# latticeboltzmann/2d-lb

Hardware: AMD Instinct MI355X
Metric: MLUPS (million lattice updates per second), fused D2Q9 BGK step (higher is better)
Workload: dtype f32

## Files before the change

### 2d-lb_amd/csrc/kernels_deep2.h

```cpp
#pragma once

namespace {

constexpr int deep2_split(int D) { return D >= 8 ? 4 : (D + 1) / 2; }
constexpr int deep2_rw_front(int D) { return deep2_split(D) - 2 >= 2 ? 2 : 1; }
constexpr int deep2_rw_back(int D) { return (D - deep2_split(D) + 1) - 2 >= 2 ? 2 : 1; }
constexpr int DEEP2_WAVES = 4;

__device__ __forceinline__ void deep2_barrier() { asm volatile("s_waitcnt lgkmcnt(0)\n\ts_barrier" ::: "memory"); }

__device__ __forceinline__ void deep2_set_prio(const StepArgs &a, const int role_mode)
{
    int mode = a.deep2_prio;
#ifdef LB_DIAG
    if ((a.diag >> 25) & 3) mode = ((a.diag >> 25) & 3) - 1;
#endif
    if (mode == role_mode) __builtin_amdgcn_s_setprio(1);
}

template <int BC, bool MASK, int F, int RW, bool DOWN, int NST>
__device__ __forceinline__ void deep2_front_fill(const StepArgs &a, const DeepCtx &cx, DeepState<RW, F - 1 - RW> &st, Row1 &ra, Row1 &rb,
                                                 int &trip)
{
    if constexpr (NST < F) {
        deep2_barrier();
        if (trip < cx.n_iter) {
            if ((NST & 1) == 0) deep_iter<BC, MASK, false, F, RW, 1, DOWN, NST, -1, DEEP_FRONT>(a, cx, NST - 1, st, rb, ra);
            else deep_iter<BC, MASK, false, F, RW, 1, DOWN, NST, -1, DEEP_FRONT>(a, cx, NST - 1, st, ra, rb);
        }
        deep2_barrier();
        ++trip;
        deep2_front_fill<BC, MASK, F, RW, DOWN, NST + 1>(a, cx, st, ra, rb, trip);
    }
}

template <int BC, bool MASK, int D, int F, int RW, bool DOWN>
__device__ __forceinline__ void deep2_front(const StepArgs &a, const int x0, const int ym, const int len, const int trips, f4a (*mine)[64],
                                            f4a (*other)[64], f4a (*ho)[64], f4a (*dma)[64])
{
    deep2_set_prio(a, 1);
    DeepCtx cx;
    cx.lane = threadIdx.x;
    const int xr = x0 + cx.lane * 4;
    cx.x4 = skirt_column<BC>(a, xr, deep_skirt_lanes(D));
    cx.store_lane = false;
    cx.ym = ym; cx.n_iter = len + D - 1;
    cx.mine = mine; cx.other = other; cx.ho = ho; cx.dma = dma;
    cx.dma_off = __builtin_amdgcn_readfirstlane((unsigned)reinterpret_cast<unsigned long long>(dma));
    DeepState<RW, F - 1 - RW> st = {};
    auto row_at = [&](int p) { return DOWN ? ym - 1 - p : ym + p; };
    Row1 ra, rb;
    deep_row_issue_lds<BC, MASK>(a, row_at(0), cx.x4, cx.dma_off, ra);
    int trip = 0;
    deep2_front_fill<BC, MASK, F, RW, DOWN, 1>(a, cx, st, ra, rb, trip);
    if ((F - 1) & 1) ra = rb;
    for (; trip < trips; ++trip) {
#ifdef LB_DIAG
        if (!(a.diag & (1 << 24)))
#endif
        deep2_barrier();
        if (trip < cx.n_iter) {
            deep_iter<BC, MASK, false, F, RW, 1, DOWN, F, -1, DEEP_FRONT>(a, cx, trip, st, ra, rb);
            ra = rb;
        }
#ifdef LB_DIAG
        if (!(a.diag & (1 << 24)))
#endif
        deep2_barrier();
    }
    asm volatile("s_waitcnt vmcnt(0)" ::: "memory");
}

template <bool MASK>
__device__ __forceinline__ void deep2_take(const DeepCtx &cx, Row1 &cur)
{
#pragma unroll
    for (int k = 0; k < 9; ++k) cur.q[k] = cx.ho[k][cx.lane];
    cur.mk = uc4{0, 0, 0, 0};
    if (MASK) cur.mk = __builtin_bit_cast(uc4, reinterpret_cast<const unsigned *>(cx.ho[9])[cx.lane]);
    cur.have = true;
}

template <int BC, bool MASK, bool MACRO, int DB, int RW, bool DOWN, int NST>
__device__ __forceinline__ void deep2_back_fill(const StepArgs &a, const DeepCtx &cx, DeepState<RW, DB - 1 - RW> &st, Row1 &cur, int &j)
{
    if constexpr (NST < DB) {
        if (j < cx.n_iter) deep2_take<MASK>(cx, cur);
        deep2_barrier();
        if (j < cx.n_iter) deep_iter<BC, MASK, MACRO, DB, RW, 0, DOWN, NST, -1, DEEP_BACK>(a, cx, NST - 1, st, cur, cur);
        deep2_barrier();
        ++j;
        deep2_back_fill<BC, MASK, MACRO, DB, RW, DOWN, NST + 1>(a, cx, st, cur, j);
    }
}

template <int BC, bool MASK, bool MACRO, int D, int F, int RW, bool DOWN>
__device__ __forceinline__ void deep2_back(const StepArgs &a, const int x0, const int ym, const int len, const int trips, f4a (*mine)[64],
                                           f4a (*other)[64], f4a (*ho)[64])
{
    constexpr int DB = D - F + 1;
    deep2_set_prio(a, 2);
    DeepCtx cx;
    cx.lane = threadIdx.x;
    const int xr = x0 + cx.lane * 4;
    cx.x4 = skirt_column<BC>(a, xr, deep_skirt_lanes(D));
    cx.store_lane = skirt_store_lane(a, cx.lane, xr, deep_skirt_lanes(D));
    cx.ym = ym; cx.n_iter = len + DB - 1;
    cx.mine = mine; cx.other = other; cx.ho = ho;
    DeepState<RW, DB - 1 - RW> st = {};
    Row1 cur;
    cur.wp = WrapPatch{0.f, 0.f, 0.f, 0.f, 0.f, 0.f};
    cur.hsolid = false; cur.hxc = -1; cur.rr = 0;
    for (int t = 0; t < F; ++t) {
        deep2_barrier();
        deep2_barrier();
    }
    int j = 0;
    deep2_back_fill<BC, MASK, MACRO, DB, RW, DOWN, 1>(a, cx, st, cur, j);
    for (; j + F < trips; ++j) {
        if (j < cx.n_iter) deep2_take<MASK>(cx, cur);
#ifdef LB_DIAG
        if (!(a.diag & (1 << 24)))
#endif
        deep2_barrier();
        if (j < cx.n_iter) deep_iter<BC, MASK, MACRO, DB, RW, 0, DOWN, DB, -1, DEEP_BACK>(a, cx, j, st, cur, cur);
#ifdef LB_DIAG
        if (!(a.diag & (1 << 24)))
#endif
        deep2_barrier();
    }
}

template <int BC, bool MASK, bool MACRO, int D>
__global__ __launch_bounds__(64 * DEEP2_WAVES, 2) void k_deep2(const StepArgs a, int strips, int seg_rows, int nsegs, int row_end)
{
    constexpr int F = deep2_split(D), RWF = deep2_rw_front(D), RWB = deep2_rw_back(D);
    constexpr int LF = (F - 1 - RWF) * DEEP_WSLOTS, LBK = (D - F - RWB) * DEEP_WSLOTS;
    static_assert(2 * (LF + LBK + 2 * DEEP_HO_SLOTS) <= 80, "two workgroups per CU: 80 KB each");
    __shared__ f4a lds_dma[2][DEEP_HO_SLOTS][64];
    __shared__ f4a lds_front[2][LF][64];
    __shared__ f4a lds_back[2][LBK][64];
    __shared__ f4a lds_ho[2][DEEP_HO_SLOTS][64];
    const int wy = (__builtin_amdgcn_readfirstlane(threadIdx.y) + ((blockIdx.x >> 8) & 1) * 2) & 3;
    const int item = xcd_item(blockIdx.x, gridDim.x);
#ifdef LB_DIAG
    const unsigned long long diag_t0 = __builtin_amdgcn_s_memrealtime();
#endif
    int sx, sy;
    if (item < strips * nsegs) {
        sx = item % strips;
        sy = item / strips;
    } else {
        if (!a.edge_seg_rows) return;
        const int j = item - strips * nsegs;
        sx = (j & 1) ? strips - 1 : 0;
        sy = nsegs + (j >> 1);
    }
    int stride = a.seg_stride;
    if (a.edge_seg_rows && (sx == 0 || sx == strips - 1)) stride = seg_rows = a.edge_seg_rows;
    const int ya = a.row_begin + sy * stride;
    if (ya >= row_end) return;
    const int yb = min(ya + seg_rows, row_end);
    const int ym = ya + (yb - ya) / 2;
    const int x0 = sx * deep_valid(D) - 4 * deep_skirt_lanes(D);
    const int trips = max(ym - ya, yb - ym) + D;
    if (wy == 0) deep2_front<BC, MASK, D, F, RWF, true>(a, x0, ym, ym - ya, trips, lds_front[0], lds_front[1], lds_ho[0], lds_dma[0]);
    else if (wy == 1) deep2_front<BC, MASK, D, F, RWF, false>(a, x0, ym, yb - ym, trips, lds_front[1], lds_front[0], lds_ho[1], lds_dma[1]);
    else if (wy == 2) deep2_back<BC, MASK, MACRO, D, F, RWB, true>(a, x0, ym, ym - ya, trips, lds_back[0], lds_back[1], lds_ho[0]);
    else deep2_back<BC, MASK, MACRO, D, F, RWB, false>(a, x0, ym, yb - ym, trips, lds_back[1], lds_back[0], lds_ho[1]);
#ifdef LB_DIAG
    if ((a.diag & 4096) && threadIdx.x == 0) {
        __builtin_amdgcn_s_waitcnt(0);
        const unsigned long long t1 = __builtin_amdgcn_s_memrealtime();
        unsigned *o = reinterpret_cast<unsigned *>(a.rho) + 8 * (item * DEEP2_WAVES + wy);
        o[0] = (unsigned)diag_t0; o[1] = (unsigned)(diag_t0 >> 32); o[2] = (unsigned)t1; o[3] = (unsigned)(t1 >> 32);
        o[4] = __builtin_amdgcn_s_getreg((31 << 11) | 20);
        o[5] = __builtin_amdgcn_s_getreg((31 << 11) | 4);
        o[6] = (unsigned)(item * DEEP2_WAVES + wy); o[7] = (unsigned)((wy & 1) ? yb - ym : ym - ya);
    }
#endif
}

}
```

### 2d-lb_amd/csrc/launch.cpp

```cpp
#include "host.h"

StepArgs step_args(const lb_sim *s, int row_begin, int row_step, int row_count)
{
    StepArgs a;
    a.src = s->origin(s->cur);
    a.dst = s->origin(s->cur ^ 1);
    a.mask = s->has_mask ? s->mask : nullptr;
    a.rho = s->rho; a.u = s->u; a.v = s->v;
    a.plane = s->plane; a.pitch = (int)s->rowp; a.fpitch = (int)s->pitch;
    a.nx = s->p.nx; a.ny = s->p.ny; a.y0 = s->p.y0; a.h = s->H;
    a.row_begin = row_begin; a.row_step = row_step; a.row_count = row_count;
    a.wrap_y = (s->p.bc_mode == LB_BC_PERIODIC && !s->multi_slab()) ? 1 : (s->p.bc_mode == LB_BC_VELOCITY_INLET ? 2 : 0);
    a.u_w = s->p.inlet_u; a.u_e = s->p.outlet_u; a.corner = s->vi_corner;
    const bool periodic = (s->p.bc_mode == LB_BC_PERIODIC);
    a.ghost_s = (s->multi_slab() && (periodic || s->p.y0 > 0)) ? 1 : 0;
    a.ghost_n = (s->multi_slab() && (periodic || s->p.y0 + s->H < s->p.ny)) ? 1 : 0;
    a.seg_stride = 0;
    a.edge_seg_rows = 0;
    a.tile_launch_order = (s->variant >= 0 && (s->variant & LB_VAR_TILE_LAUNCH_ORDER)) ? 1 : 0;
    a.diag = s->diag;
    a.prio_turns = 0;
    a.deep2_prio = 0;
    a.nts = 0;
    a.omega = s->p.omega; a.rho_in = s->p.inlet_rho; a.rho_out = s->p.outlet_rho;
    a.lid_u = s->p.lid_u; a.rho0 = s->p.rho0;
    return a;
}

int launch_step(lb_sim *s, int row_begin, int row_step, int row_count, bool macro)
{
    if (row_count <= 0) return LB_OK;
    macro = macro && !lazy_macro(s);
    const StepArgs a = step_args(s, row_begin, row_step, row_count);
    const int variant = effective_variant(s);
    const int rpb_sel = variant & LB_VAR_ROWS;
    const int rows_per_block = rpb_sel == LB_VAR_ROWS_1 ? 1 : (rpb_sel == LB_VAR_ROWS_2 ? 2 : 4);
    const int waves_x = 4 / rows_per_block;
    dim3 block(64 * waves_x, rows_per_block);
    const int lanes_x = (int)(s->pitch / 4);
    dim3 grid((lanes_x + block.x - 1) / block.x, (row_count + rows_per_block - 1) / rows_per_block);
    lbk_launch_step(kernel_bc(s), s->has_mask, macro, variant, grid, block, s->stream, a);
    HIP_TRY(hipGetLastError());
    return LB_OK;
}

static bool launch_march(const lb_sim *s, hipStream_t st, const StepArgs &a, const MarchPlan &m, int row_end, bool macro, int depth)
{
    const int waves = (depth >= 4) ? STEP4_WAVES : 4;
    MarchLaunch g;
    g.block = dim3(64, waves);
    g.grid = dim3(depth >= 4 ? m.items : (m.items + waves - 1) / waves);
    g.stream = st;
    g.strips = m.strips; g.seg_rows = m.seg_rows; g.nsegs = m.segs; g.row_end = row_end;
    const int bc = kernel_bc(s);
    if (depth == 7 && deep2_chosen(s)) return lbk_launch_deep2_7(bc, s->has_mask, macro, g, a);
    if (depth == 7) return lbk_launch_deep7(bc, s->has_mask, macro, g, a);
    if (depth == 6) return lbk_launch_deep6(bc, s->has_mask, macro, g, a);
    if (depth == 5) lbk_launch_march5(bc, s->has_mask, macro, g, a);
    else if (depth == 4) lbk_launch_march4(bc, s->has_mask, macro, !(effective_variant(s) & LB_VAR_STEP4_NO_AHEAD), g, a);
    else lbk_launch_march23(depth, bc, s->has_mask, macro, g, a);
    return true;
}

constexpr int DEEP2_PRIO = 2;

int launch_marching(lb_sim *s, const MarchRows &r)
{
    if (r.row_end <= r.row_begin) return LB_OK;
    const bool macro = r.macro && !lazy_macro(s);
    StepArgs a = step_args(s, r.row_begin, 1, r.row_end - r.row_begin);
    const int variant = effective_variant(s);
    const MarchPlan m = plan_march(s, r.row_end - r.row_begin, r.depth, r.bands, r.reserve);
    a.seg_stride = m.seg_stride;
    a.edge_seg_rows = m.edge_seg_rows;
    a.prio_turns = (variant & LB_VAR_NO_PRIO_TURNS) ? 0 : 13;
    a.deep2_prio = DEEP2_PRIO;
    a.nts = (variant & LB_VAR_NT_STORES) ? 1 : 0;
    if (!launch_march(s, r.stream, a, m, r.row_end, macro, r.depth))
        return fail(LB_ERR_STATE, "no %d-step kernel for this boundary family (the caller's schedule must not ask for one)", r.depth);
    HIP_TRY(hipGetLastError());
    return LB_OK;
}

static int launch_tile4(lb_sim *s, bool macro)
{
    macro = macro && !lazy_macro(s);
    const StepArgs a = step_args(s, 0, 1, s->H);
    if (!lbk_launch_tile4(kernel_bc(s), s->has_mask, macro, tile_shape_of(s), s->p.nx, s->H, s->stream, a))
        return fail(LB_ERR_STATE, "no LDS-tile kernel for this boundary family");
    HIP_TRY(hipGetLastError());
    return LB_OK;
}

constexpr int GRAPH_STEPS = 16;

void drop_graph(lb_sim *s)
{
    if (s->graph_exec) (void)hipGraphExecDestroy(s->graph_exec);
    if (s->graph) (void)hipGraphDestroy(s->graph);
    s->graph_exec = nullptr;
    s->graph = nullptr;
    s->graph_key = -1;
}

static int ensure_graph(lb_sim *s)
{
    const int key = (s->cur & 1) | (s->has_mask ? 2 : 0) | (effective_variant(s) << 2);
    if (s->graph_exec && s->graph_key == key && s->graph_stream == s->stream) return LB_OK;
    if (s->graph_failed) return LB_OK;
    drop_graph(s);
    if (hipStreamBeginCapture(s->stream, hipStreamCaptureModeRelaxed) != hipSuccess) {
        (void)hipGetLastError();
        s->graph_failed = true;
        return LB_OK;
    }
    int rc = LB_OK;
    const int cur0 = s->cur;
    for (int i = 0; i < GRAPH_STEPS && !rc; ++i) {
        rc = launch_step(s, 0, 1, s->H, false);
        s->cur ^= 1;
    }
    s->cur = cur0;
    hipGraph_t g = nullptr;
    const hipError_t e = hipStreamEndCapture(s->stream, &g);
    if (rc || e != hipSuccess || !g || hipGraphInstantiate(&s->graph_exec, g, nullptr, nullptr, 0) != hipSuccess) {
        (void)hipGetLastError();
        if (g) (void)hipGraphDestroy(g);
        s->graph_exec = nullptr;
        s->graph_failed = true;
        return LB_OK;
    }
    s->graph = g;
    s->graph_key = key;
    s->graph_stream = s->stream;
    return LB_OK;
}

static int vel_band_pass(lb_sim *s, int d, bool macro)
{
    int rc;
    const int H = s->H;
    const hipStream_t q = s->edge_stream;
    HIP_TRY(hipEventRecord(s->ev_interior, s->stream));
    HIP_TRY(hipStreamWaitEvent(q, s->ev_interior, 0));
    const StepArgs a = step_args(s, 0, 1, H);
    const dim3 grid((unsigned)((s->p.nx + (64 - 2 * d) - 1) / (64 - 2 * d))), blk(256);
    lbk_launch_vel_band(s->has_mask, macro, d, grid, blk, q, a);
    HIP_TRY(hipGetLastError());
    MarchRows interior;
    interior.stream = s->stream; interior.row_begin = d; interior.row_end = H - d; interior.depth = d; interior.macro = macro;
    if ((rc = launch_marching(s, interior))) return rc;
    HIP_TRY(hipEventRecord(s->ev_boundary, q));
    HIP_TRY(hipStreamWaitEvent(s->stream, s->ev_boundary, 0));
    return LB_OK;
}

int run_whole_grid(lb_sim *s, int n_steps, bool final_macro)
{
    int rc;
    const int depths = whole_grid_depths(s);
    const bool tile = use_tile_kernel(s);
    int left = n_steps;
    if (depths == depth_mask(false, false) && left > GRAPH_STEPS && small_grid(s)) {
        if ((rc = ensure_graph(s))) return rc;
        while (s->graph_exec && left > GRAPH_STEPS) {
            HIP_TRY(hipGraphLaunch(s->graph_exec, s->stream));
            left -= GRAPH_STEPS;
        }
    }
    const bool store_macro = final_macro && !lazy_macro(s);
    while (left > 0) {
        const int adv = next_advance(s, depths, left);
        const bool macro = store_macro && (left == adv);
        if (adv == 4 && tile) rc = launch_tile4(s, macro);
        else if (adv >= 3 && s->p.bc_mode == LB_BC_VELOCITY_INLET) rc = vel_band_pass(s, adv, macro);
        else if (adv >= 2) {
            MarchRows all;
            all.stream = s->stream; all.row_begin = 0; all.row_end = s->H; all.depth = adv; all.macro = macro;
            rc = launch_marching(s, all);
        }
        else rc = launch_step(s, 0, 1, s->H, macro);
        if (rc) return rc;
        s->cur ^= 1;
        left -= adv;
    }
    if (n_steps) {
        s->feq_valid = false;
        s->macro_valid = store_macro || !lazy_macro(s) || (s->diag & 4096);
    }
    return LB_OK;
}

int run_scalar(lb_sim *s, int n_steps)
{
    const AdExtra e = ad_extra(s);
    int left = n_steps;
    while (left > 0) {
        const int adv = scalar_next_advance(s, left);
        const StepArgs a = step_args(s, 0, 1, s->H);
        if (adv == TILE_T) lbk_ad_tile4(s->p.bc_mode, s->ad_G != 0.f, left == adv, scalar_tile_shape(s), s->stream, a, e);
        else lbk_ad_step(s->p.bc_mode, s->ad_G != 0.f, left == adv, s->stream, a, e);
        HIP_TRY(hipGetLastError());
        s->cur ^= 1;
        left -= adv;
    }
    if (n_steps) { s->feq_valid = false; s->macro_valid = true; }
    return LB_OK;
}

int run_poisson(lb_sim *s, int n_steps)
{
    PsExtra e = ps_extra(s);
    for (int it = 0; it < n_steps; ++it) {
        e.store_rho = it == n_steps - 1;
        lbk_ps_step(false, s->stream, step_args(s, 0, 1, s->H), e);
        HIP_TRY(hipGetLastError());
        s->cur ^= 1;
    }
    s->ps_iter += n_steps;
    if (n_steps) { s->feq_valid = false; s->macro_valid = true; }
    return LB_OK;
}

int run_porous(lb_sim *s, int n_steps)
{
    const PmExtra e = pm_extra(s);
    for (int it = 0; it < n_steps; ++it) {
        lbk_pm_step(s->p.bc_mode, it == n_steps - 1, s->stream, step_args(s, 0, 1, s->H), e);
        HIP_TRY(hipGetLastError());
        s->cur ^= 1;
    }
    if (n_steps) { s->feq_valid = false; s->macro_valid = true; }
    return LB_OK;
}
```

Measured before the change: 500,200.

## Assign deep2 wave roles by hardware SIMD id and prioritize front waves

Instead of mapping wave index to front/back role statically, each wave reads its SIMD id from the HW_ID register, publishes it in LDS, and roles are assigned so that each role lands on a distinct SIMD (falling back to the static map if SIMDs are not all distinct). The intent is to spread the two producer (front) and two consumer (back) waves evenly across SIMDs to balance issue contention. It also switches elevated wave priority from the back waves to the front waves. This adds an extra barrier and LDS round trip at kernel start.

Measured after the change: 522,600 (median of 6 runs). 4.5% higher.

```diff
diff --git a/2d-lb_amd/csrc/deep2_roles.h b/2d-lb_amd/csrc/deep2_roles.h
--- /dev/null
+++ b/2d-lb_amd/csrc/deep2_roles.h
@@ -0,0 +1,19 @@
+#pragma once
+
+#if defined(__HIPCC__) || defined(__CUDACC__)
+#define DEEP2_ROLES_FN __host__ __device__ inline
+#else
+#define DEEP2_ROLES_FN inline
+#endif
+
+DEEP2_ROLES_FN int deep2_static_role(int w, int flip) { return (w + 2 * flip) & 3; }
+
+DEEP2_ROLES_FN void deep2_assign_roles(const int simd[4], int flip, int role[4])
+{
+    flip &= 1;
+    unsigned seen = 0;
+    for (int w = 0; w < 4; ++w)
+        if (simd[w] >= 0 && simd[w] < 4) seen |= 1u << simd[w];
+    const bool by_simd = seen == 15u;
+    for (int w = 0; w < 4; ++w) role[w] = by_simd ? ((simd[w] + 2 * flip) & 3) : deep2_static_role(w, flip);
+}
diff --git a/2d-lb_amd/csrc/kernels_deep2.h b/2d-lb_amd/csrc/kernels_deep2.h
--- a/2d-lb_amd/csrc/kernels_deep2.h
+++ b/2d-lb_amd/csrc/kernels_deep2.h
@@ -1,4 +1,6 @@
 #pragma once
+
+#include "deep2_roles.h"
 
 namespace {
 
@@ -131,6 +133,38 @@
     }
 }
 
+__device__ __forceinline__ int deep2_take_role(const StepArgs &a, unsigned *lds_role, unsigned &note)
+{
+    const int w = __builtin_amdgcn_readfirstlane(threadIdx.y);
+    const int launch_flip = (blockIdx.x >> 8) & 1;
+    int sig = 1;
+#ifdef LB_DIAG
+    if (a.diag & (1 << 27)) {
+        note = (unsigned)launch_flip << 30;
+        return deep2_static_role(w, launch_flip);
+    }
+    if ((a.diag >> 28) & 3) sig = (a.diag >> 28) & 3;
+#endif
+    const unsigned hw = __builtin_amdgcn_s_getreg((31 << 11) | 4);
+    unsigned word = (hw >> 4) & 3u;
+    if (sig == 2) word |= (hw & 1u) << 2;
+    if (sig == 3) word |= (__builtin_amdgcn_s_getreg((31 << 11) | 6) & 0xfffu) ? 4u : 0u;
+    if (threadIdx.x == 0) lds_role[w] = word;
+    deep2_barrier();
+    int simd[DEEP2_WAVES], role[DEEP2_WAVES];
+    unsigned word0 = 0;
+#pragma unroll
+    for (int k = 0; k < DEEP2_WAVES; ++k) {
+        const unsigned v = __builtin_amdgcn_readfirstlane(lds_role[k]);
+        simd[k] = (int)(v & 3u);
+        if (k == 0) word0 = v;
+    }
+    const int flip = sig == 1 ? launch_flip : (int)((word0 >> 2) & 1u);
+    deep2_assign_roles(simd, flip, role);
+    note = ((unsigned)flip << 30) | (1u << 29);
+    return w == 0 ? role[0] : (w == 1 ? role[1] : (w == 2 ? role[2] : role[3]));
+}
+
 template <int BC, bool MASK, bool MACRO, int D>
 __global__ __launch_bounds__(64 * DEEP2_WAVES, 2) void k_deep2(const StepArgs a, int strips, int seg_rows, int nsegs, int row_end)
 {
@@ -141,7 +175,7 @@
     __shared__ f4a lds_front[2][LF][64];
     __shared__ f4a lds_back[2][LBK][64];
     __shared__ f4a lds_ho[2][DEEP_HO_SLOTS][64];
-    const int wy = (__builtin_amdgcn_readfirstlane(threadIdx.y) + ((blockIdx.x >> 8) & 1) * 2) & 3;
+    __shared__ unsigned lds_role[DEEP2_WAVES];
     const int item = xcd_item(blockIdx.x, gridDim.x);
 #ifdef LB_DIAG
     const unsigned long long diag_t0 = __builtin_amdgcn_s_memrealtime();
@@ -164,6 +198,8 @@
     const int ym = ya + (yb - ya) / 2;
     const int x0 = sx * deep_valid(D) - 4 * deep_skirt_lanes(D);
     const int trips = max(ym - ya, yb - ym) + D;
+    unsigned role_note = 0;
+    const int wy = deep2_take_role(a, lds_role, role_note);
     if (wy == 0) deep2_front<BC, MASK, D, F, RWF, true>(a, x0, ym, ym - ya, trips, lds_front[0], lds_front[1], lds_ho[0], lds_dma[0]);
     else if (wy == 1) deep2_front<BC, MASK, D, F, RWF, false>(a, x0, ym, yb - ym, trips, lds_front[1], lds_front[0], lds_ho[1], lds_dma[1]);
     else if (wy == 2) deep2_back<BC, MASK, MACRO, D, F, RWB, true>(a, x0, ym, ym - ya, trips, lds_back[0], lds_back[1], lds_ho[0]);
@@ -176,9 +212,9 @@
         o[0] = (unsigned)diag_t0; o[1] = (unsigned)(diag_t0 >> 32); o[2] = (unsigned)t1; o[3] = (unsigned)(t1 >> 32);
         o[4] = __builtin_amdgcn_s_getreg((31 << 11) | 20);
         o[5] = __builtin_amdgcn_s_getreg((31 << 11) | 4);
-        o[6] = (unsigned)(item * DEEP2_WAVES + wy); o[7] = (unsigned)((wy & 1) ? yb - ym : ym - ya);
-    }
-#endif
-}
-
-}
+        o[6] = (unsigned)(item * DEEP2_WAVES + wy); o[7] = (unsigned)((wy & 1) ? yb - ym : ym - ya) | role_note;
+    }
+#endif
+}
+
+}
diff --git a/2d-lb_amd/csrc/launch.cpp b/2d-lb_amd/csrc/launch.cpp
--- a/2d-lb_amd/csrc/launch.cpp
+++ b/2d-lb_amd/csrc/launch.cpp
@@ -62,7 +62,7 @@
     return true;
 }
 
-constexpr int DEEP2_PRIO = 2;
+constexpr int DEEP2_PRIO = 1;
 
 int launch_marching(lb_sim *s, const MarchRows &r)
 {
```
